# SauersML/genomic_pca

Hardware: AMD Instinct MI355X
Metric: SNPs x samples / sec through rSVD at k=20; max|dPC| vs ref (higher is better)
Workload: dtype i8 (exact: int8 dosages x 4 signed 7-bit fixed-point digit planes of the skinny operand, i32 accumulate, f64 recombination; accuracy >= f32)

## Files before the change

genomic_pca_amd/csrc/gpca_internal.h:

```cpp
#pragma once
#include "../../include/gpca.h"
#include "kernels.h"

#include <dlfcn.h>
#include <hip/hip_runtime.h>

#include <algorithm>
#include <atomic>
#include <chrono>
#include <condition_variable>
#include <deque>
#include <thread>
#include <cmath>
#include <cstdio>
#include <cstdlib>
#include <cstring>
#include <map>
#include <mutex>
#include <string>
#include <vector>

using namespace gpca;

typedef struct ncclComm* ncclComm_t;
// ... 79 lines not shown
    int device = 0;
    int precision = GPCA_PREC_I8_EXACT;
    int storage = GPCA_STORE_INT8;
    int storage_cfg = GPCA_STORE_AUTO;
    int nd_cfg = 0;
    int auto_pin = 0;
    hipStream_t st = nullptr;
    std::string err;

    int64_t M = 0, N = 0, ldg = 0, Mpad = 0;
    int64_t ld8 = 0;
    int64_t cap_rows_pad = 0;
    int64_t cap_stats_pad = 0;
    int8_t* dG = nullptr;
    uint8_t* dG2 = nullptr;
    int64_t ld2 = 0;
    uint32_t pack_flags = 0;

    bool have_stats = false;
    float *d_mu = nullptr, *d_sigma = nullptr, *d_r = nullptr, *d_b = nullptr;
    uint8_t *d_keep = nullptr, *d_reason = nullptr;
    uint32_t *d_counts = nullptr, *d_flags = nullptr;
    int64_t n_pca = 0;
    std::vector<int64_t> pca_rows;
    int64_t* d_pca_rows = nullptr;
    uint32_t flags = 0;

    int k = 0, l = 0, L = 0;
    bool have_rsvd = false;
    float *dQ = nullptr, *dT = nullptr, *dTb = nullptr, *dYpart = nullptr, *d_cpart = nullptr, *d_s32 = nullptr;
    double* h_pin = nullptr;
    int spin_sync = 1;
    int* d_cholflag = nullptr;
    double *d_scratch64 = nullptr, *dY = nullptr, *d_c = nullptr, *d_part64 = nullptr, *dW = nullptr, *dZ = nullptr, *d_s64 = nullptr;
    double* d_tr64 = nullptr; size_t cap_tr64 = 0;
    double* d_scores64 = nullptr; float* d_scores32 = nullptr; float* d_load32 = nullptr; int* d_sign = nullptr;
    double* d_eigres = nullptr;
    double* d_cand_val = nullptr; int64_t* d_cand_idx = nullptr;
    size_t cap_Q = 0, cap_T = 0, cap_Tb = 0, cap_Ypart = 0, cap_cpart = 0, cap_Y = 0, cap_part64 = 0, cap_scores = 0, cap_load = 0;
    std::vector<double> eig, sv;
    GttPlan plan{};
    GqPlan gqplan{};
    Gtt8Plan plan8{};
    int8_t *dQd = nullptr, *dTd = nullptr;
    bool c_fold_pending = false;
    double* d_apart = nullptr; size_t cap_apart = 0; bool apart_valid = false; int64_t apart_parts = 0;
    const double* apart_src[4] = {nullptr, nullptr, nullptr, nullptr};
    float* d_rmax = nullptr; bool rmax_valid = false;
    double* d_amax_run = nullptr;
    double* d_yint = nullptr; size_t cap_yint = 0;
    uint8_t* d_smask = nullptr;
    int64_t n_smask = 0;
    float* d_cw = nullptr; int32_t* d_cfeat0 = nullptr; int c_cmax = 0; int64_t c_R = 0; int c_B = 0;
    int64_t *d_cblk_row0 = nullptr, *d_cblk_row1 = nullptr; int32_t *d_cblk_feat0 = nullptr, *d_cblk_c = nullptr;
    double* dP = nullptr; size_t cap_P = 0;
    float* d_lqr = nullptr; size_t cap_lqr = 0;
    float *d_ones = nullptr, *d_zeros = nullptr; size_t cap_ones = 0, cap_zeros = 0;
    bool loadings_valid = true;
    double* d_status = nullptr;
    double* h_status = nullptr;
    hipEvent_t ev_status = nullptr;
    std::string status_own;
    struct PullLane {
        hipStream_t st = nullptr;
        hipEvent_t dep = nullptr;
        int64_t *d_rows = nullptr, *d_cols = nullptr; float* d_out = nullptr; unsigned long long* d_err = nullptr;
// ... 215 lines not shown
```

genomic_pca_amd/csrc/gpca_residency.cpp:

```cpp
#include "gpca_internal.h"

using namespace gpca;

void free_stats(gpca_handle* h) {
    dfree(h->d_mu); dfree(h->d_sigma); dfree(h->d_r); dfree(h->d_b); dfree(h->d_keep); dfree(h->d_reason);
    dfree(h->d_counts); dfree(h->d_flags); dfree(h->d_pca_rows);
    h->have_stats = false; h->n_pca = 0; h->pca_rows.clear(); h->cap_stats_pad = 0;
}
void free_eigensnp(gpca_handle* h) {
    dfree(h->d_smask); h->n_smask = 0; dfree(h->d_cw); dfree(h->d_cfeat0); dfree(h->d_cblk_row0); dfree(h->d_cblk_row1); dfree(h->d_cblk_feat0); dfree(h->d_cblk_c);
    dfree(h->dP); dfree(h->d_lqr); dfree(h->d_ones); dfree(h->d_zeros);
    h->cap_P = h->cap_lqr = h->cap_ones = h->cap_zeros = 0; h->c_cmax = 0; h->c_R = 0; h->c_B = 0; h->loadings_valid = true;
}
void free_ws(gpca_handle* h) {
    free_eigensnp(h);
    dfree(h->dQ); dfree(h->dT); dfree(h->dTb); dfree(h->dYpart); dfree(h->d_cpart); dfree(h->d_s32); dfree(h->dY); dfree(h->d_c);
    dfree(h->d_part64); dfree(h->dW); dfree(h->dZ); dfree(h->d_s64); dfree(h->d_scores64); dfree(h->d_scores32);
    dfree(h->d_load32); dfree(h->d_sign); dfree(h->d_eigres); dfree(h->d_cand_val); dfree(h->d_cand_idx); dfree(h->d_scratch64); dfree(h->d_tr64); h->cap_tr64 = 0;
    dfree(h->dQd); dfree(h->dTd); dfree(h->dYpart64); dfree(h->d_apart); h->cap_apart = 0; dfree(h->d_cholflag); if (h->h_pin) { (void)hipHostFree(h->h_pin); h->h_pin = nullptr; } dfree(h->d_qscale); dfree(h->d_qinv); dfree(h->d_tscale); dfree(h->d_tinv);
    dfree(h->d_amax_run); dfree(h->d_rmax); h->rmax_valid = false; dfree(h->d_yint); h->cap_yint = 0;
    h->cap_Qd = h->cap_Td = h->cap_Ypart64 = 0;
    h->cap_Q = h->cap_T = h->cap_Tb = h->cap_Ypart = h->cap_cpart = h->cap_Y = h->cap_part64 = h->cap_scores = h->cap_load = 0;
    h->have_rsvd = false;
}
static inline bool host_kind(int kind) { return kind == GPCA_PANEL_HOST_I8 || kind == GPCA_PANEL_HOST_BED || kind == GPCA_PANEL_MAPPED_I8 || kind == GPCA_PANEL_MAPPED_BED; }
static inline bool bed_kind(int kind) { return kind == GPCA_PANEL_HOST_BED || kind == GPCA_PANEL_MAPPED_BED; }
static inline bool mapped_kind(int kind) { return kind == GPCA_PANEL_MAPPED_I8 || kind == GPCA_PANEL_MAPPED_BED; }
static inline double ms_since(std::chrono::steady_clock::time_point t0) {
    return std::chrono::duration<double, std::milli>(std::chrono::steady_clock::now() - t0).count();
}

static void copy_mapped_rows(const Filler& f, int64_t row0, int64_t rows, void* dst) {
    const int64_t w = f.stage_ld;
    const int T = (int)std::max<int64_t>(1, std::min<int64_t>(f.copy_threads, rows * w / (4 << 20)));
    auto part = [&](int t) {
        const int64_t a = rows * t / T, b = rows * (t + 1) / T;
        const uint8_t* src = f.map_base + (size_t)(row0 + a) * (size_t)f.map_ld;
        uint8_t* d = (uint8_t*)dst + (size_t)a * (size_t)w;
        if (f.map_ld == w) memcpy(d, src, (size_t)(b - a) * (size_t)w);
        else for (int64_t r = a; r < b; ++r, src += f.map_ld, d += w) memcpy(d, src, (size_t)w);
    };
    if (T == 1) { part(0); return; }
    std::vector<std::thread> th;
    for (int t = 1; t < T; ++t) th.emplace_back(part, t);
    part(0);
    for (auto& x : th) x.join();
}

static void filler_worker(Filler* f) {
    (void)hipSetDevice(f->device);
    std::unique_lock<std::mutex> lk(f->m);
    for (;;) {
        f->cv.wait(lk, [&] { return f->quit || (!f->jobs.empty() && f->st_state[(size_t)(f->produced % (uint64_t)f->n_stage)] != Filler::kReady); });
        if (f->quit) return;
        const size_t b = (size_t)(f->produced % (uint64_t)f->n_stage);
        const std::pair<int64_t, int64_t> job = f->jobs.front();
// ... 589 lines not shown
```

genomic_pca_amd/csrc/gpca_rsvd.cpp:

```cpp
#include "gpca_internal.h"

using namespace gpca;

static void tred2(int n, double* V, double* d, double* e) {
    for (int j = 0; j < n; ++j) d[j] = V[(n - 1) * n + j];
    for (int i = n - 1; i > 0; --i) {
        double scale = 0.0, h = 0.0;
        for (int k = 0; k < i; ++k) scale += std::fabs(d[k]);
        if (scale == 0.0) {
            e[i] = d[i - 1];
            for (int j = 0; j < i; ++j) { d[j] = V[(i - 1) * n + j]; V[i * n + j] = 0.0; V[j * n + i] = 0.0; }
        } else {
            for (int k = 0; k < i; ++k) { d[k] /= scale; h += d[k] * d[k]; }
            double f = d[i - 1];
            double g = std::sqrt(h);
            if (f > 0) g = -g;
            e[i] = scale * g; h -= f * g; d[i - 1] = f - g;
            for (int j = 0; j < i; ++j) e[j] = 0.0;
            for (int j = 0; j < i; ++j) {
                f = d[j]; V[j * n + i] = f; g = e[j] + V[j * n + j] * f;
                for (int k = j + 1; k <= i - 1; ++k) { g += V[k * n + j] * d[k]; e[k] += V[k * n + j] * f; }
                e[j] = g;
            }
            f = 0.0;
// ... 346 lines not shown
        HIPCHK(hipGetLastError());
    }
    const bool i8 = h->precision == GPCA_PREC_I8_EXACT;
    const int64_t tparts = tail_num_parts(h->ldg);
    const double* csum_part = h->d_part64;
    const double* amax_part = h->d_part64 + tparts * L;
    if (i8 && tparts <= kFinishQFoldMax) {
        for (int hf = 0; hf < L / 32; ++hf) {
            launch_quantize_f64_finishq(h->st, h->dY + 32 * hf, h->N, h->ldg, h->dQd + (size_t)hf * h->ldg * 32 * kDigits, h->storage == GPCA_STORE_2BIT ? 1 : 0, h->nd, L,
                                        csum_part + 32 * hf, amax_part + 32 * hf, tparts, L, h->d_s64 + 32 * hf, h->d_s32 + 32 * hf, h->d_qscale + 32 * hf, h->d_qinv + 32 * hf);
            HIPCHK(hipGetLastError());
        }
        return GPCA_OK;
    }
    launch_finish_q(h->st, csum_part, amax_part, tparts, L, h->d_s64, h->d_s32, i8 ? h->d_qscale : nullptr, i8 ? h->d_qinv : nullptr, h->nd);
    HIPCHK(hipGetLastError());
    if (i8) {
        for (int hf = 0; hf < L / 32; ++hf) {
            launch_quantize_f64_prescaled(h->st, h->dY + 32 * hf, h->N, h->ldg, h->d_qinv + 32 * hf, h->dQd + (size_t)hf * h->ldg * 32 * kDigits,
                                          h->storage == GPCA_STORE_2BIT ? 1 : 0, h->nd, L);
            HIPCHK(hipGetLastError());
        }
    }
    return GPCA_OK;
}

static int ensure_workspace(gpca_handle* h) {
    const int L = h->L;
    const int64_t Npad = h->ldg, M = h->M, N = h->N;
    const int64_t gemm_rows = h->sm.on ? h->sm.panel_rows : h->Mpad;
    h->plan = gtt_plan(h->Mpad, Npad, L, h->gtt_waves_target);
    h->gqplan = k1_plan(h, gemm_rows);
    CHK(ensure(h, h->dQ, h->cap_Q, (size_t)Npad * L));
    CHK(ensure(h, h->dT, h->cap_T, (size_t)h->Mpad * L));
    if (h->precision == GPCA_PREC_F32_MFMA) CHK(ensure(h, h->dTb, h->cap_Tb, (size_t)h->Mpad * L));
    if (h->Mpad > M) HIPCHK(hipMemsetAsync(h->dT + (size_t)M * L, 0, (size_t)(h->Mpad - M) * L * 4, h->st));
    if (h->precision == GPCA_PREC_F32_MFMA) CHK(ensure(h, h->dYpart, h->cap_Ypart, (size_t)h->plan.W * (size_t)Npad * L));
    const int64_t cparts = cpart_capacity(h->gqplan.waves, h->Mpad, L);
    CHK(ensure(h, h->d_cpart, h->cap_cpart, (size_t)cparts));
    CHK(ensure(h, h->dY, h->cap_Y, (size_t)N * L + 16));
    const int64_t p64 = part64_capacity(M, h->Mpad, N, Npad, L);
    CHK(ensure(h, h->d_part64, h->cap_part64, (size_t)p64));
    if (!h->d_c) {
        constexpr size_t LL = (size_t)kMaxSketch * kMaxSketch;
        HIPCHK(hipMalloc((void**)&h->d_c, kMaxSketch * 8)); HIPCHK(hipMalloc((void**)&h->d_s64, kMaxSketch * 8));
        HIPCHK(hipMalloc((void**)&h->d_s32, kMaxSketch * 4)); HIPCHK(hipMalloc((void**)&h->dW, (LL + 16) * 8));
        HIPCHK(hipMalloc((void**)&h->dZ, 2 * LL * 8));
        HIPCHK(hipHostMalloc((void**)&h->h_pin, (3 * LL + 16) * 8, hipHostMallocDefault)); HIPCHK(hipMalloc((void**)&h->d_sign, kMaxSketch * 4));
        HIPCHK(hipMalloc((void**)&h->d_scratch64, (size_t)sum_scratch_capacity(kMaxSketch) * 8));
        HIPCHK(hipMalloc((void**)&h->d_eigres, kEigResCount * 8));
        HIPCHK(hipMalloc((void**)&h->d_cand_val, (size_t)scores_cand_capacity() * 8)); HIPCHK(hipMalloc((void**)&h->d_cand_idx, (size_t)scores_cand_capacity() * 8));
        HIPCHK(hipMalloc((void**)&h->d_cholflag, 4));
    }
    if (h->precision == GPCA_PREC_I8_EXACT) {
        h->plan8 = k2_plan(h, gemm_rows);
        CHK(ensure(h, h->dQd, h->cap_Qd, (size_t)Npad * 32 * kDigits * (size_t)(L / 32)));
        CHK(ensure(h, h->dTd, h->cap_Td, (size_t)h->Mpad * 32 * kDigits * (size_t)(L / 32)));
        int64_t yslices = h->plan8.W;
        if (h->sm.on && h->M % h->sm.panel_rows) yslices = std::max<int64_t>(yslices, k2_plan(h, round_up(h->M % h->sm.panel_rows, kGQRowsPerWave)).W);
        CHK(ensure(h, h->dYpart64, h->cap_Ypart64, (size_t)yslices * (size_t)Npad * 32));
        CHK(ensure(h, h->d_apart, h->cap_apart, (size_t)h->gqplan.waves * 32 * (size_t)(L / 32)));
        if (h->sm.on) CHK(ensure(h, h->d_yint, h->cap_yint, (size_t)N * 32 * (size_t)(L / 32)));
        if (!h->d_qscale) {
            HIPCHK(hipMalloc((void**)&h->d_qscale, kMaxSketch * 8)); HIPCHK(hipMalloc((void**)&h->d_qinv, kMaxSketch * 8));
            HIPCHK(hipMalloc((void**)&h->d_tscale, kMaxSketch * 8)); HIPCHK(hipMalloc((void**)&h->d_tinv, kMaxSketch * 8));
            HIPCHK(hipMalloc((void**)&h->d_amax_run, kMaxSketch * 8));
            HIPCHK(hipMalloc((void**)&h->d_rmax, 4));
        }
    }
    size_t cap2 = h->cap_scores;
    CHK(ensure(h, h->d_scores64, h->cap_scores, (size_t)N * h->k));
    CHK(ensure(h, h->d_scores32, cap2, (size_t)N * h->k));
    CHK(ensure(h, h->d_load32, h->cap_load, (size_t)std::max<int64_t>(h->n_pca, 1) * h->k));
    return GPCA_OK;
}

static int rsvd_preflight(gpca_handle* h, int32_t k, int32_t oversample, int32_t power_iters) {
    if (!have_genotypes(h)) return fail(h, GPCA_ERR_STATE, "gpca_rsvd: no genotypes resident and no panel stream open");
    if (!h->have_stats) return fail(h, GPCA_ERR_STATE, "gpca_rsvd: run gpca_snp_stats or gpca_set_standardization first");
    if (k <= 0) return fail(h, GPCA_ERR_BAD_ARG, "Number of components (-k) must be > 0.");
    if (oversample < 0 || power_iters < 0) return fail(h, GPCA_ERR_BAD_ARG, "gpca_rsvd: negative oversample/power_iters");
    if (h->N < 2) return fail(h, GPCA_ERR_BAD_ARG, "PCA requires at least 2 samples.");
    if (!multi_rank(h) && h->n_pca == 0) return fail(h, GPCA_ERR_BAD_ARG, "PCA requires at least 1 variant (feature), found 0.");
    const int l = k + oversample;
    if (l > kMaxSketch) return fail(h, GPCA_ERR_BAD_ARG, "gpca_rsvd: k + oversample must be <= 128");
    if (l > 64 && h->precision != GPCA_PREC_I8_EXACT)
        return fail(h, GPCA_ERR_BAD_ARG, "gpca_rsvd: sketches wider than 64 columns (k + oversample > 64) run on GPCA_PREC_I8_EXACT; GPCA_PREC_F32_MFMA holds up to 64");
    if (l > h->N || (!multi_rank(h) && l > h->n_pca)) return fail(h, GPCA_ERR_BAD_ARG, "gpca_rsvd: k + oversample exceeds min(samples, PCA SNPs)");
    if (h->flags & 1u) return fail(h, GPCA_ERR_MISSING_GENOTYPE,
        "Unexpected missing genotype (-127i8) in a PCA SNP. This should have been filtered by QC.");
    if (h->flags & 2u) return fail(h, GPCA_ERR_INVALID_GENOTYPE, "a PCA SNP holds a dosage outside {0,1,2}");
    if (h->sm.on && h->precision != GPCA_PREC_I8_EXACT) return fail(h, GPCA_ERR_STATE, "gpca_rsvd: streamed panels need GPCA_PREC_I8_EXACT");
    if (h->precision == GPCA_PREC_I8_EXACT && h->N > ((int64_t)1 << 22))
        return fail(h, GPCA_ERR_BAD_ARG, "gpca_rsvd: the exact-integer path holds up to 4 194 304 samples per matrix (i32 accumulators); use GPCA_PREC_F32_MFMA beyond");
    HIPCHK(hipSetDevice(h->device));
    h->k = k; h->l = l; h->L = l <= 32 ? 32 : (l <= 64 ? 64 : kMaxSketch);
    h->have_rsvd = false;
    CHK(ensure_workspace(h));
    HIPCHK(hipMemsetAsync(h->d_cholflag, 0, 4, h->st));
    return GPCA_OK;
}

static int enqueue_small_eigh(gpca_handle* h, const double* src, int nslices, int zmode, double denom) {
    launch_small_eigh(h->st, src, nslices, h->l, h->L, h->k, zmode, denom, h->d_cholflag, h->dZ, h->d_eigres, nullptr);
    HIPCHK(hipGetLastError());
    return GPCA_OK;
}
static int enqueue_scores_loadings(gpca_handle* h, const float* Xload, bool loadings) {
    const int L = h->L, k = h->k;
    const size_t zk = (size_t)L * k;
    if (L <= 64) {
        launch_scores(h->st, h->dY, h->N, L, h->dZ, k, h->d_scores64, h->d_cand_val, h->d_cand_idx);
        HIPCHK(hipGetLastError());
        launch_scores_sign(h->st, h->d_scores64, h->d_scores32, h->N, k, h->d_cand_val, h->d_cand_idx, scores_num_parts(h->N), h->d_sign);
        HIPCHK(hipGetLastError());
        if (loadings) launch_rightmul_gather_f32(h->st, Xload, h->d_pca_rows, h->n_pca, L, h->dZ + zk, k, h->d_load32, h->d_sign);
    } else {
        launch_rightmul_f64(h->st, h->dY, h->N, L, h->dZ, k, h->d_scores64, (float*)nullptr);
        HIPCHK(hipGetLastError());
        launch_col_sign(h->st, h->d_scores64, h->N, k, h->d_sign);
        launch_scale_cols(h->st, h->d_scores64, h->d_scores32, h->N, k, h->d_sign);
        HIPCHK(hipGetLastError());
        if (loadings) {
            launch_scale_cols(h->st, h->dZ + zk, (float*)nullptr, L, k, h->d_sign);
            launch_rightmul_gather_f32(h->st, Xload, h->d_pca_rows, h->n_pca, L, h->dZ + zk, k, h->d_load32);
        }
    }
    HIPCHK(hipGetLastError());
    return GPCA_OK;
}
static int finish_small_eigh(gpca_handle* h, bool take) {
    double* res = h->h_pin;
    HIPCHK(hipMemcpyAsync(res, h->d_eigres, sizeof(double) * kEigResCount, hipMemcpyDeviceToHost, h->st));
    HIPCHK(stream_wait(h));
    if (!take) return GPCA_OK;
    static_assert(kEigNotConverged == GPCA_ERR_NOT_CONVERGED, "eig_result.h restates the status code");
    const EigVerdict verdict = eig_result_verdict(res, h->l);
    if (verdict.status != 0) return fail(h, verdict.status, verdict.msg);
    h->sv.assign(res + kEigResSv, res + kEigResSv + h->l);
    h->eig.assign(res + kEigResEig, res + kEigResEig + h->k);
    return GPCA_OK;
}

static int call_tail(gpca_handle* h, int zmode, double denom, const float* Xload, int lrc) {
    const bool mr = multi_rank(h);
    const int L = h->L;
    const double* gsrc = h->dW; int gslices = 0;
    auto gram = [&]() -> int {
        const int64_t rows = zmode == 0 ? h->M : h->N;
        const int64_t parts = gram_num_parts(rows);
        if (zmode == 0) launch_gram_f32(h->st, h->dT, rows, L, h->d_part64);
        else launch_gram_f64(h->st, h->dY, rows, L, h->d_part64);
        HIPCHK(hipGetLastError());
        if (mr) launch_sum_partials_f64(h->st, h->d_part64, parts, (int64_t)L * L, h->dW, h->d_scratch64);
        else launch_sum_partials_f64_stage1(h->st, h->d_part64, parts, (int64_t)L * L, h->d_scratch64, &gsrc, &gslices);
        HIPCHK(hipGetLastError());
        return GPCA_OK;
    };
    LOCAL(gram());
    if (mr) {
        h->status_own = h->err;
        status_histogram(h->h_status, lrc);
        if (hipMemcpyAsync(h->dW + (size_t)L * L, h->h_status, 16 * sizeof(double), hipMemcpyHostToDevice, h->st) != hipSuccess && lrc == GPCA_OK)
            lrc = fail(h, GPCA_ERR_HIP, "gpca_rsvd: status copy failed");
        const int xrc = allreduce_f64(h, h->dW, (int64_t)L * L + 16);
        if (xrc != GPCA_OK) return xrc;
    }
// ... 492 lines not shown
```

genomic_pca_amd/csrc/kernels.h:

```cpp
#pragma once
#include <hip/hip_runtime.h>
#include <stdint.h>
#include "eig_result.h"
#include "plan_math.h"

namespace gpca {

struct QcParams { double min_call_rate, min_maf, max_hwe_p; };

struct KernelOpts {
    int gq_phase = -1;
    int gq_chain = 1;
    int gtt_xcd = 1;
};
int init_device_kernels_i8();
int init_device_kernels_common();
int init_device_kernels_eig();

void launch_small_eigh(hipStream_t st, const double* src, int nslices, int n, int L, int k, int zmode, double denom, const int* cholflag,
                       double* Z, double* res, double* Vout);

template <class T>
__host__ __device__ inline constexpr T acc_row(T row0, int e, int h) { return row0 + (e & 3) + 8 * (e >> 2) + 4 * h; }

__host__ __device__ inline int64_t blocked_t_index(int64_t row, int col, int LT) {
    const int64_t group = row >> 4;
    const int w = (int)(row & 15), lt = col >> 5, cc = col & 31;
    return ((group * LT + lt) * 64 + ((w & 1) * 32 + cc)) * 8 + (w >> 1);
}
__host__ __device__ inline int64_t blocked_q_index(int64_t n, int col, int LT) {
    const int64_t chunk = n >> 5;
    const int w = (int)(n & 31), lt = col >> 5, cc = col & 31;
    return ((chunk * LT + lt) * 64 + ((w >> 4) * 32 + cc)) * 16 + (w & 15);
}

void launch_synth(hipStream_t st, int8_t* G, int64_t M, int64_t N, int64_t ld, int64_t snp_offset,
                  uint64_t seed, const uint32_t* d_thresh, int P);
void launch_synth16(hipStream_t st, void* G, int packed, int64_t rows, int64_t N, int64_t ld, int64_t snp0, uint64_t seed,
                    const uint32_t* d_thresh16, int P);
void launch_bed_decode(hipStream_t st, const uint8_t* bed, int64_t bytes_per_row, int8_t* G, int64_t M,
                       int64_t N, int64_t ld);
void launch_snp_stats(hipStream_t st, const int8_t* G, int64_t M, int64_t N, int64_t ld, QcParams qc,
                      float* mu, float* sigma, float* r, float* b, uint8_t* keep, uint8_t* reason,
                      uint32_t* counts, uint32_t* flags);
void launch_set_scale(hipStream_t st, int64_t M, const float* mu, const float* sigma, const uint8_t* keep,
                      float* r, float* b);
void launch_standardize_block(hipStream_t st, const int8_t* G, int64_t ld, const float* mu,
                              const float* sigma, const int64_t* rows, int64_t ns, const int64_t* cols,
                              int64_t nj, float* out, unsigned long long* err_idx);

void launch_omega(hipStream_t st, int64_t M, int64_t Mpad, int l, int L, int64_t snp_offset, uint64_t seed,
                  const float* r, const float* b, float* Tb, float* cpart, double* apart, int blocked = 1, const int64_t* row_ids = nullptr);
// ... 194 lines not shown
```

genomic_pca_amd/csrc/kernels.hip:

```cpp
#include "kernels.h"
#include "philox.hpp"
#include "omega_math.h"

#ifndef GPCA_OMEGA_ABLATE
#define GPCA_OMEGA_ABLATE 0
#endif
namespace gpca {

__device__ const OmegaLnEntry kOmegaLnTable[kOmegaLnEntries] = {
#include "omega_table.inc"
};

typedef float f32x16 __attribute__((ext_vector_type(16)));

#define DEVINL __device__ __forceinline__

__global__ __launch_bounds__(256) void k_synth(int8_t* __restrict__ G, int64_t M, int64_t N, int64_t ld,
                                                int64_t snp_offset, uint64_t seed,
                                                const uint32_t* __restrict__ thresh, int P) {
    const int64_t per_row = ld >> 3;
    const int64_t t = (int64_t)blockIdx.x * 256 + threadIdx.x;
    if (t >= M * per_row) return;
    const int64_t i = t / per_row;
    const int64_t n0 = (t - i * per_row) << 3;
// ... 804 lines not shown
    const int total = (int)rows_here * K;
    float* dst = out32 + n0 * K;
    for (int e = threadIdx.x; e < total; e += 256) dst[e] = osm[(e / K) * KP + (e % K)];
}
static size_t rightmul_lds(int L, int K, bool f32out) { return sizeof(double) * L * K + (f32out ? sizeof(float) * 256 * (size_t)(K | 1) : 0); }
void launch_rightmul_f64(hipStream_t st, const double* X, int64_t rows, int L, const double* Z, int K, double* out64,
                         float* out32) {
    const dim3 grid((unsigned)((rows + 255) / 256)), blk(256);
    const size_t lds = rightmul_lds(L, K, out32 != nullptr);
    if (L == 32) hipLaunchKernelGGL((k_rightmul<double, 32>), grid, blk, lds, st, X, (const int64_t*)nullptr, rows, Z, K, out64, out32);
    else if (L == 64) {
        hipLaunchKernelGGL((k_rightmul<double, 64>), grid, blk, lds, st, X, (const int64_t*)nullptr, rows, Z, K, out64, out32);
    } else launch_rightmul_any_f64(st, X, rows, L, Z, K, out64, out32);
}
template <int L, int NJ>
__global__ __launch_bounds__(256) void k_rightmul_mfma(const float* __restrict__ X, const int64_t* __restrict__ row_ids,
                                                       int64_t nrows, const double* __restrict__ Z, int K,
                                                       float* __restrict__ out32, int64_t tiles_per_wave, const int* __restrict__ sign) {
    constexpr int E = L / 4;
    const int lane = threadIdx.x & 63, wv = threadIdx.x >> 6;
    const int i = lane & 15, kq = lane >> 4;
    double zb[E][NJ];
#pragma unroll
    for (int jt = 0; jt < NJ; ++jt) {
        const int col = 16 * jt + i;
        const double sg = (sign && col < K) ? (double)sign[col] : 1.0;
#pragma unroll
        for (int s2 = 0; s2 < E; ++s2) zb[s2][jt] = col < K ? Z[(E * kq + s2) * K + col] * sg : 0.0;
    }
    __shared__ float osm[4][16 * 64];
    const int64_t ntiles = (nrows + 15) >> 4;
    const int64_t t0 = ((int64_t)blockIdx.x * 4 + wv) * tiles_per_wave;
    const int64_t t1 = (t0 + tiles_per_wave < ntiles) ? t0 + tiles_per_wave : ntiles;
    float xa[E], xn[E];
    auto load_tile = [&](int64_t tile, float (&dst)[E]) {
        const int64_t row = tile * 16 + i;
        const bool valid = row < nrows && tile < t1;
        const int64_t src = valid ? (row_ids ? row_ids[row] : row) : 0;
        const float4* xp = reinterpret_cast<const float4*>(X + src * L + E * kq);
#pragma unroll
        for (int v = 0; v < E / 4; ++v) {
            const float4 q = xp[v];
            dst[4 * v] = valid ? q.x : 0.f; dst[4 * v + 1] = valid ? q.y : 0.f; dst[4 * v + 2] = valid ? q.z : 0.f; dst[4 * v + 3] = valid ? q.w : 0.f;
        }
    };
    if (t0 < t1) load_tile(t0, xa);
    for (int64_t tile = t0; tile < t1; ++tile) {
        load_tile(tile + 1, xn);
        f64x4 acc[NJ];
#pragma unroll
        for (int jt = 0; jt < NJ; ++jt) acc[jt] = f64x4{0.0, 0.0, 0.0, 0.0};
#pragma unroll
        for (int s2 = 0; s2 < E; ++s2) {
            const double a = (double)xa[s2];
#pragma unroll
            for (int jt = 0; jt < NJ; ++jt) acc[jt] = __builtin_amdgcn_mfma_f64_16x16x4f64(a, zb[s2][jt], acc[jt], 0, 0, 0);
        }
#pragma unroll
        for (int jt = 0; jt < NJ; ++jt) {
            const int col = 16 * jt + i;
            if (col < K) {
#pragma unroll
                for (int r = 0; r < 4; ++r) osm[wv][(4 * r + kq) * K + col] = (float)acc[jt][r];
            }
        }
        const int64_t rows_here = (nrows - tile * 16 < 16) ? nrows - tile * 16 : 16;
        float* dst = out32 + tile * 16 * K;
        for (int e = lane; e < (int)rows_here * K; e += 64) dst[e] = osm[wv][e];
#pragma unroll
        for (int s2 = 0; s2 < E; ++s2) xa[s2] = xn[s2];
    }
}
void launch_rightmul_gather_f32(hipStream_t st, const float* X, const int64_t* row_ids, int64_t nrows, int L,
                                const double* Z, int K, float* out32, const int* sign) {
    if (nrows == 0) return;
    if (L > 64) { launch_rightmul_any_gather_f32(st, X, row_ids, nrows, L, Z, K, out32); return; }
    const int64_t ntiles = (nrows + 15) / 16;
    int64_t tpw = ntiles / (4 * 2048);
    if (tpw < 1) tpw = 1;
    const int64_t waves = (ntiles + tpw - 1) / tpw;
    const dim3 grid((unsigned)((waves + 3) / 4)), blk(256);
    const int nj = (K + 15) / 16;
#define GPCA_RM(LL, NN) hipLaunchKernelGGL((k_rightmul_mfma<LL, NN>), grid, blk, 0, st, X, row_ids, nrows, Z, K, out32, tpw, sign)
    if (L == 32) { if (nj == 1) GPCA_RM(32, 1); else if (nj == 2) GPCA_RM(32, 2); else if (nj == 3) GPCA_RM(32, 3); else GPCA_RM(32, 4); }
    else { if (nj == 1) GPCA_RM(64, 1); else if (nj == 2) GPCA_RM(64, 2); else if (nj == 3) GPCA_RM(64, 3); else GPCA_RM(64, 4); }
#undef GPCA_RM
}

template <int L>
__global__ __launch_bounds__(256) void k_scores(const double* __restrict__ X, int64_t nrows, const double* __restrict__ Z, int K,
                                                double* __restrict__ out64, double* __restrict__ cand_val, int64_t* __restrict__ cand_idx) {
    extern __shared__ double zsc[];
    double* tile = zsc + L * K;
    double* win_val = tile + 256 * 17;
    long long* win_idx = reinterpret_cast<long long*>(win_val + 64);
    __shared__ double seg_val[256];
    __shared__ int seg_row[256];
    for (int e = threadIdx.x; e < L * K; e += 256) zsc[e] = Z[e];
    if (threadIdx.x < 64) { win_val[threadIdx.x] = 0.0; win_idx[threadIdx.x] = -1; }
    __syncthreads();
    const int64_t nchunks = (nrows + 255) / 256;
    for (int64_t chunk = blockIdx.x; chunk < nchunks; chunk += gridDim.x) {
        const int64_t n0 = chunk * 256, n = n0 + threadIdx.x;
        const bool live = n < nrows;
        double x[L];
#pragma unroll
        for (int j = 0; j < L; ++j) x[j] = live ? X[n * L + j] : 0.0;
        for (int k0 = 0; k0 < K; k0 += 16) {
            const int kn = K - k0 < 16 ? K - k0 : 16;
            for (int kc = 0; kc < kn; ++kc) {
                double a = 0.0;
#pragma unroll
// ... 270 lines not shown
```

genomic_pca_amd/csrc/small_eig.hip:

```cpp
#include "kernels.h"

#ifndef GPCA_EIG_ABL
#define GPCA_EIG_ABL 0
#endif
#ifndef GPCA_EIG_STAMP
#define GPCA_EIG_STAMP 0
#endif
#if GPCA_EIG_STAMP
__device__ unsigned long long g_eig_stamp[20];
#define EIG_STAMP(SLOT) { if (threadIdx.x == 0) { g_eig_stamp[2 * (SLOT)] = __builtin_amdgcn_s_memrealtime(); g_eig_stamp[2 * (SLOT) + 1] = __builtin_amdgcn_s_memtime(); } }
#define EIG_COUNT(X) (++(X))
#else
#define EIG_STAMP(SLOT)
#define EIG_COUNT(X) ((void)(X))
#endif

namespace gpca {

#define EIGDEV __device__ __forceinline__
EIGDEV double eig_rsqrt(double x) {
    const double y = __builtin_amdgcn_rsq(x);
    const double h = fma(-(x * y), y, 1.0);
    return fma(y * h, fma(0.375, h, 0.5), y);
}
// ... 2 lines not shown
    double r = __builtin_amdgcn_rcp(x);
    r = fma(r, fma(-x, r, 1.0), r);
    return fma(r, fma(-x, r, 1.0), r);
}

constexpr double kJacSkip = 1e-17, kJacDone = 2e-15;
template <int L> struct JacCfg {
    static constexpr int H = L / 2;
    static constexpr int NT = L == 32 ? 256 : 1024;
    static constexpr int NBK = H * H / NT;
    static constexpr int LP = L + 2;
    static constexpr bool DB = L <= 64;
    static constexpr int NBUF = DB ? 4 : 1;
};
EIGDEV int jac_dest(int s, int Le) { return s >= Le ? s : (s == 0 ? 0 : (s == 1 ? (Le > 2 ? 2 : 1) : ((s & 1) ? s - 2 : (s == Le - 2 ? Le - 1 : s + 2)))); }
template <int L> EIGDEV int jac_at(int r, int c) { return r * JacCfg<L>::LP + ((r >> 1) & 1) + c; }

EIGDEV void jac_rot(double app, double a01, double a10, double aqq, double& c, double& s) {
    const double b2 = a01 + a10, dd = aqq - app;
#if GPCA_EIG_ABL & 1
    c = 0.8; s = 0.6; return;
#endif
    const bool live = fabs(b2) > 2.0 * kJacSkip;
    const double sq = live ? fma(dd, dd, b2 * b2) : 1.0;
    const double rinv = eig_rsqrt(sq);
    const double c2 = fabs(dd) * rinv, s2 = (dd >= 0.0 ? b2 : -b2) * rinv;
    const double h = fma(0.5, c2, 0.5);
    const double ci = eig_rsqrt(h);
    c = live ? h * ci : 1.0; s = live ? 0.5 * s2 * ci : 0.0;
}

template <int NT, class GetV>
EIGDEV void eig_emit(GetV getV, double* wsl, int* order, const int* genuine, int slots, int n, int Lw, int k, int zmode, double denom, double unsc,
                     const int* __restrict__ cholflag, int capped, double* __restrict__ Z, double* __restrict__ res, double* __restrict__ Vout, int tid) {
    double wmine = 0.0; int rank = -1;
    if (tid < slots && genuine[tid]) {
        wmine = wsl[tid]; rank = 0;
        for (int t = 0; t < slots; ++t) { const double wt = wsl[t]; if (t != tid && genuine[t] && (wt > wmine || (wt == wmine && t < tid))) ++rank; }
    }
    __syncthreads();
    if (rank >= 0 && rank < n) { order[rank] = tid; wsl[rank] = wmine; }
    __syncthreads();
    for (int j = tid; j < kMaxSketchCols; j += NT) {
        const double w = j < n ? wsl[j] * unsc : 0.0;
        res[kEigResW + j] = w;
        res[kEigResSv + j] = w > 0.0 ? sqrt(w) : 0.0;
        res[kEigResEig + j] = j < k ? w / denom : 0.0;
    }
    if (tid == 0) { res[kEigResFlag] = cholflag ? (double)cholflag[0] : 0.0; res[kEigResFlag + 1] = (double)capped; }
    for (int e0 = tid; e0 < Lw * k; e0 += NT) {
        const int r = e0 / k, c = e0 - r * k;
        double z0 = 0.0, z1 = 0.0;
        if (r < n && c < n) {
            const double x = getV(r, order[c]);
            if (zmode == 0) {
                const double w = wsl[c] * unsc;
                const double sv = w > 0.0 ? sqrt(w) : 0.0;
                z0 = x * sv; z1 = sv > 0.0 ? x / sv : 0.0;
            } else { z0 = x; z1 = x; }
        }
        Z[e0] = z0; Z[(size_t)Lw * k + e0] = z1;
    }
    EIG_STAMP(4)
    if (Vout)
        for (int e0 = tid; e0 < n * n; e0 += NT) { const int r = e0 / n, c = e0 - r * n; Vout[e0] = getV(r, order[c]); }
}

template <int L>
__global__ __launch_bounds__(JacCfg<L>::NT) void k_small_eigh(const double* __restrict__ src, int nslices, int n, int Lw, int k, int zmode, double denom,
                                                             const int* __restrict__ cholflag, double* __restrict__ Z, double* __restrict__ res,
                                                             double* __restrict__ Vout) {
    using C = JacCfg<L>;
    constexpr int H = C::H, NT = C::NT, NBK = C::NBK, LP = C::LP, BUF = L * LP;
    extern __shared__ double eig_sm[];
    __shared__ double wsl[128];
    __shared__ int order[128], genuine[128];
    __shared__ double redmax[NT];
    const int tid = threadIdx.x;
#if GPCA_EIG_STAMP
    if (tid == 0) { g_eig_stamp[10] = 0; g_eig_stamp[11] = 0; }
#endif
    EIG_STAMP(0)
    const int S = nslices > 0 ? nslices : 1;
    const size_t LL = (size_t)Lw * Lw;
    double* buf0 = eig_sm;
    for (int e0 = tid; e0 < BUF; e0 += NT) buf0[e0] = 0.0;
    __syncthreads();
    for (int e0 = tid; e0 < n * n; e0 += 4 * NT) {
        const double* p[4];
        double acc[4] = {0.0, 0.0, 0.0, 0.0};
#pragma unroll
        for (int q = 0; q < 4; ++q) { const int e1 = e0 + NT * q; const int e2 = e1 < n * n ? e1 : e0; p[q] = src + (size_t)(e2 / n) * Lw + (e2 % n); }
        for (int s0 = 0; s0 < S; s0 += 8) {
            double v[4][8];
#pragma unroll
            for (int u = 0; u < 8; ++u) {
                const int sl = s0 + u < S ? s0 + u : s0;
#pragma unroll
                for (int q = 0; q < 4; ++q) v[q][u] = p[q][sl * LL];
            }
#pragma unroll
            for (int u = 0; u < 8; ++u)
#pragma unroll
// ... 139 lines not shown
    static constexpr int RING = 512;
    static constexpr int NCONS = L / 64;
    static constexpr int kDoubles = L * L + 6 * L + 64 + 2 * RING;
    static constexpr size_t kBytes = sizeof(double) * kDoubles + sizeof(int) * (RING + 16);
};
template <int L> EIGDEV int ql_at(int r, int c) { return r * L + ((c + r) & (L - 1)); }
EIGDEV int ql_tag(int seq) { return (((seq >> 9) + 1) & 0xffff) << 12; }
template <int CTRL, int ROWMASK> EIGDEV double eig_dpp0(double v) {
    const int hi = __builtin_amdgcn_update_dpp(0, __double2hiint(v), CTRL, ROWMASK, 0xf, true);
    const int lo = __builtin_amdgcn_update_dpp(0, __double2loint(v), CTRL, ROWMASK, 0xf, true);
    return __hiloint2double(hi, lo);
}
EIGDEV double eig_lane(double v, int i) {
    return __hiloint2double(__builtin_amdgcn_readlane(__double2hiint(v), i), __builtin_amdgcn_readlane(__double2loint(v), i));
}
EIGDEV double wave_sum(double x) {
    x += eig_dpp0<0x111, 0xf>(x); x += eig_dpp0<0x112, 0xf>(x); x += eig_dpp0<0x114, 0xf>(x); x += eig_dpp0<0x118, 0xf>(x);
    x += eig_dpp0<0x142, 0xa>(x); x += eig_dpp0<0x143, 0xc>(x);
    return eig_lane(x, 63);
}
EIGDEV double oct_sum(double x) {
    x += eig_dpp0<0xb1, 0xf>(x);
    x += eig_dpp0<0x4e, 0xf>(x);
    x += eig_dpp0<0x141, 0xf>(x);
    return x;
}
EIGDEV double wave_max(double x) { for (int o = 32; o > 0; o >>= 1) x = fmax(x, __shfl_xor(x, o)); return x; }
constexpr int kQlFirst = 1 << 30, kQlLast = 1 << 29, kQlDoneFlag = 1 << 28, kQlIndex = 0xff, kQlTagMask = 0xffff << 12;
constexpr int kQlSpinCap = 4000000;
enum { kQlTail0 = 2, kQlTail1 = 3, kQlGaveUp = 4 };

template <int L>
__global__ __launch_bounds__(QlCfg<L>::NT) void k_small_eigh_ql(const double* __restrict__ src, int nslices, int n, int Lw, int k, int zmode, double denom,
                                                                const int* __restrict__ cholflag, double* __restrict__ Z, double* __restrict__ res,
                                                                double* __restrict__ Vout) {
    using C = QlCfg<L>;
    constexpr int NT = C::NT, RING = C::RING;
    extern __shared__ double eig_sm[];
    typedef __attribute__((address_space(3))) double lds_d;
    typedef __attribute__((address_space(3))) int lds_i;
    typedef double v2d __attribute__((ext_vector_type(2)));
    typedef __attribute__((address_space(3))) v2d lds_d2;
    lds_d* A = (lds_d*)eig_sm;
    lds_d* de = A + L * L;
    lds_d* vv = A + L * L + 2 * L;
    lds_d* pp = vv + L;
    lds_d* ww = pp + L;
    lds_d* bb = ww + L;
    lds_d* red = bb + L;
    volatile lds_d2* ringcs = (volatile lds_d2*)(red + 64);
    volatile lds_i* ringi = (volatile lds_i*)(red + 64 + 2 * RING);
    volatile lds_i* ctrl = ringi + RING;
    __shared__ double wsl[128];
    __shared__ int order[128], genuine[128];
    const int tid = threadIdx.x, lane = tid & 63, wave = tid >> 6;
    EIG_STAMP(0)
    const int S = nslices > 0 ? nslices : 1;
    const size_t LL = (size_t)Lw * Lw;
    for (int e0 = tid; e0 < L * L; e0 += NT) A[e0] = 0.0;
    if (tid < 16) ctrl[tid] = 0;
    for (int e0 = tid; e0 < RING; e0 += NT) ringi[e0] = 0;
    if (tid < 128) { order[tid] = 0; genuine[tid] = tid < n; }
    __syncthreads();
    for (int e0 = tid; e0 < n * n; e0 += NT) {
        const int r = e0 / n, c = e0 - r * n;
        const double* p0 = src + (size_t)r * Lw + c;
        double acc = 0.0;
// ... 271 lines not shown
                carry = hi;
            }
            tail += len; EIG_COUNT(batches);
            if ((tail & 63) < len && lane == 0) ctrl[kQlTail0 + wave - 1] = tail;
        }
#if GPCA_EIG_STAMP
        if (wave == 1 && lane == 0) { g_eig_stamp[13] = (unsigned long long)batches; g_eig_stamp[14] = (unsigned long long)empty_polls; }
#endif
        (void)batches; (void)empty_polls;
    }
    __syncthreads();
    capped = ctrl[kQlGaveUp] != 0 || (wave == 0 && capped);
    if (wave == 0 && lane == 0 && capped) ctrl[kQlGaveUp] = 1;
    __syncthreads();
    capped = ctrl[kQlGaveUp];
    EIG_STAMP(3)
    if (tid < 128) wsl[tid] = tid < n ? de[2 * tid] : 0.0;
    __syncthreads();
    eig_emit<NT>([&](int r, int slot) { return A[ql_at<L>(r, slot)]; }, wsl, order, genuine, L, n, Lw, k, zmode, denom, unsc, cholflag, capped, Z, res, Vout, tid);
}

template <int L> static size_t small_eigh_lds() { return sizeof(double) * (size_t)L * JacCfg<L>::LP * JacCfg<L>::NBUF; }
#ifndef GPCA_EIG_QL
#define GPCA_EIG_QL 1
#endif
int init_device_kernels_eig() {
    hipError_t e = hipFuncSetAttribute(reinterpret_cast<const void*>(k_small_eigh<128>), hipFuncAttributeMaxDynamicSharedMemorySize, (int)small_eigh_lds<128>());
    if (e == hipSuccess) e = hipFuncSetAttribute(reinterpret_cast<const void*>(k_small_eigh_ql<128>), hipFuncAttributeMaxDynamicSharedMemorySize, (int)QlCfg<128>::kBytes);
    if (e == hipSuccess) e = hipFuncSetAttribute(reinterpret_cast<const void*>(k_small_eigh_ql<64>), hipFuncAttributeMaxDynamicSharedMemorySize, (int)QlCfg<64>::kBytes);
    if (e == hipSuccess) e = hipFuncSetAttribute(reinterpret_cast<const void*>(k_small_eigh<64>), hipFuncAttributeMaxDynamicSharedMemorySize, (int)small_eigh_lds<64>());
    if (e == hipSuccess) e = hipFuncSetAttribute(reinterpret_cast<const void*>(k_small_eigh<32>), hipFuncAttributeMaxDynamicSharedMemorySize, (int)small_eigh_lds<32>());
    return (int)e;
}
void launch_small_eigh(hipStream_t st, const double* src, int nslices, int n, int L, int k, int zmode, double denom, const int* cholflag,
                       double* Z, double* res, double* Vout) {
    if (n <= 32) hipLaunchKernelGGL(k_small_eigh<32>, dim3(1), dim3(JacCfg<32>::NT), small_eigh_lds<32>(), st, src, nslices, n, L, k, zmode, denom, cholflag, Z, res, Vout);
    else if (GPCA_EIG_QL == 2 && n <= 64) hipLaunchKernelGGL(k_small_eigh_ql<64>, dim3(1), dim3(QlCfg<64>::NT), QlCfg<64>::kBytes, st, src, nslices, n, L, k, zmode, denom, cholflag, Z, res, Vout);
    else if (GPCA_EIG_QL && n > 64) hipLaunchKernelGGL(k_small_eigh_ql<128>, dim3(1), dim3(QlCfg<128>::NT), QlCfg<128>::kBytes, st, src, nslices, n, L, k, zmode, denom, cholflag, Z, res, Vout);
    else if (n <= 64) hipLaunchKernelGGL(k_small_eigh<64>, dim3(1), dim3(JacCfg<64>::NT), small_eigh_lds<64>(), st, src, nslices, n, L, k, zmode, denom, cholflag, Z, res, Vout);
    else hipLaunchKernelGGL(k_small_eigh<128>, dim3(1), dim3(JacCfg<128>::NT), small_eigh_lds<128>(), st, src, nslices, n, L, k, zmode, denom, cholflag, Z, res, Vout);
}

}
```

Before: 965.6 billion.

## Skip redundant per-call memsets and deepen gather-rightmul prefetch

The eig kernel now clears the Cholesky flag itself after reading it, so the per-call memset of that flag can be skipped once a completed eig run is known. The zero-fill of T's padding rows is cached and redone only when the buffer or its shape changes. The gather right-multiply kernel now prefetches two tiles ahead instead of one and uses a different tiles-per-wave split. These cut small launches per call and hide load latency, at the cost of extra state tracking and registers.

```diff
diff --git a/genomic_pca_amd/csrc/gpca_internal.h b/genomic_pca_amd/csrc/gpca_internal.h
--- a/genomic_pca_amd/csrc/gpca_internal.h
+++ b/genomic_pca_amd/csrc/gpca_internal.h
@@ -135,6 +135,8 @@
     double* h_pin = nullptr;
     int spin_sync = 1;
     int* d_cholflag = nullptr;
+    bool cholflag_zero = false, cholflag_eig_enqueued = false;
+    int64_t tpad_M = -1, tpad_Mpad = -1; int tpad_L = 0;
     double *d_scratch64 = nullptr, *dY = nullptr, *d_c = nullptr, *d_part64 = nullptr, *dW = nullptr, *dZ = nullptr, *d_s64 = nullptr;
     double* d_tr64 = nullptr; size_t cap_tr64 = 0;
     double* d_scores64 = nullptr; float* d_scores32 = nullptr; float* d_load32 = nullptr; int* d_sign = nullptr;
diff --git a/genomic_pca_amd/csrc/gpca_residency.cpp b/genomic_pca_amd/csrc/gpca_residency.cpp
--- a/genomic_pca_amd/csrc/gpca_residency.cpp
+++ b/genomic_pca_amd/csrc/gpca_residency.cpp
@@ -22,6 +22,7 @@
     h->cap_Qd = h->cap_Td = h->cap_Ypart64 = 0;
     h->cap_Q = h->cap_T = h->cap_Tb = h->cap_Ypart = h->cap_cpart = h->cap_Y = h->cap_part64 = h->cap_scores = h->cap_load = 0;
     h->have_rsvd = false;
+    h->cholflag_zero = false; h->tpad_M = -1;
 }
 static inline bool host_kind(int kind) { return kind == GPCA_PANEL_HOST_I8 || kind == GPCA_PANEL_HOST_BED || kind == GPCA_PANEL_MAPPED_I8 || kind == GPCA_PANEL_MAPPED_BED; }
 static inline bool bed_kind(int kind) { return kind == GPCA_PANEL_HOST_BED || kind == GPCA_PANEL_MAPPED_BED; }
diff --git a/genomic_pca_amd/csrc/gpca_rsvd.cpp b/genomic_pca_amd/csrc/gpca_rsvd.cpp
--- a/genomic_pca_amd/csrc/gpca_rsvd.cpp
+++ b/genomic_pca_amd/csrc/gpca_rsvd.cpp
@@ -402,9 +402,17 @@
     h->plan = gtt_plan(h->Mpad, Npad, L, h->gtt_waves_target);
     h->gqplan = k1_plan(h, gemm_rows);
     CHK(ensure(h, h->dQ, h->cap_Q, (size_t)Npad * L));
-    CHK(ensure(h, h->dT, h->cap_T, (size_t)h->Mpad * L));
+    {
+        const float* T_was = h->dT; const size_t cap_was = h->cap_T;
+        CHK(ensure(h, h->dT, h->cap_T, (size_t)h->Mpad * L));
+        if (h->dT != T_was || h->cap_T != cap_was) h->tpad_M = -1;
+    }
     if (h->precision == GPCA_PREC_F32_MFMA) CHK(ensure(h, h->dTb, h->cap_Tb, (size_t)h->Mpad * L));
-    if (h->Mpad > M) HIPCHK(hipMemsetAsync(h->dT + (size_t)M * L, 0, (size_t)(h->Mpad - M) * L * 4, h->st));
+    if (h->Mpad > M && !(h->tpad_M == M && h->tpad_Mpad == h->Mpad && h->tpad_L == L)) {
+        h->tpad_M = -1;
+        HIPCHK(hipMemsetAsync(h->dT + (size_t)M * L, 0, (size_t)(h->Mpad - M) * L * 4, h->st));
+        h->tpad_M = M; h->tpad_Mpad = h->Mpad; h->tpad_L = L;
+    }
     if (h->precision == GPCA_PREC_F32_MFMA) CHK(ensure(h, h->dYpart, h->cap_Ypart, (size_t)h->plan.W * (size_t)Npad * L));
     const int64_t cparts = cpart_capacity(h->gqplan.waves, h->Mpad, L);
     CHK(ensure(h, h->d_cpart, h->cap_cpart, (size_t)cparts));
@@ -467,13 +475,15 @@
     h->k = k; h->l = l; h->L = l <= 32 ? 32 : (l <= 64 ? 64 : kMaxSketch);
     h->have_rsvd = false;
     CHK(ensure_workspace(h));
-    HIPCHK(hipMemsetAsync(h->d_cholflag, 0, 4, h->st));
+    if (!h->cholflag_zero) HIPCHK(hipMemsetAsync(h->d_cholflag, 0, 4, h->st));
+    h->cholflag_zero = false; h->cholflag_eig_enqueued = false;
     return GPCA_OK;
 }
 
 static int enqueue_small_eigh(gpca_handle* h, const double* src, int nslices, int zmode, double denom) {
     launch_small_eigh(h->st, src, nslices, h->l, h->L, h->k, zmode, denom, h->d_cholflag, h->dZ, h->d_eigres, nullptr);
     HIPCHK(hipGetLastError());
+    h->cholflag_eig_enqueued = true;
     return GPCA_OK;
 }
 static int enqueue_scores_loadings(gpca_handle* h, const float* Xload, bool loadings) {
@@ -503,6 +513,7 @@
     double* res = h->h_pin;
     HIPCHK(hipMemcpyAsync(res, h->d_eigres, sizeof(double) * kEigResCount, hipMemcpyDeviceToHost, h->st));
     HIPCHK(stream_wait(h));
+    if (h->cholflag_eig_enqueued) h->cholflag_zero = true;
     if (!take) return GPCA_OK;
     static_assert(kEigNotConverged == GPCA_ERR_NOT_CONVERGED, "eig_result.h restates the status code");
     const EigVerdict verdict = eig_result_verdict(res, h->l);
diff --git a/genomic_pca_amd/csrc/kernels.h b/genomic_pca_amd/csrc/kernels.h
--- a/genomic_pca_amd/csrc/kernels.h
+++ b/genomic_pca_amd/csrc/kernels.h
@@ -17,7 +17,7 @@
 int init_device_kernels_common();
 int init_device_kernels_eig();
 
-void launch_small_eigh(hipStream_t st, const double* src, int nslices, int n, int L, int k, int zmode, double denom, const int* cholflag,
+void launch_small_eigh(hipStream_t st, const double* src, int nslices, int n, int L, int k, int zmode, double denom, int* cholflag,
                        double* Z, double* res, double* Vout);
 
 template <class T>
diff --git a/genomic_pca_amd/csrc/kernels.hip b/genomic_pca_amd/csrc/kernels.hip
--- a/genomic_pca_amd/csrc/kernels.hip
+++ b/genomic_pca_amd/csrc/kernels.hip
@@ -860,21 +860,31 @@
     const int64_t ntiles = (nrows + 15) >> 4;
     const int64_t t0 = ((int64_t)blockIdx.x * 4 + wv) * tiles_per_wave;
     const int64_t t1 = (t0 + tiles_per_wave < ntiles) ? t0 + tiles_per_wave : ntiles;
-    float xa[E], xn[E];
-    auto load_tile = [&](int64_t tile, float (&dst)[E]) {
+    float xa[E], xb[E], xc[E];
+    auto tile_src = [&](int64_t tile) -> int64_t {
         const int64_t row = tile * 16 + i;
-        const bool valid = row < nrows && tile < t1;
-        const int64_t src = valid ? (row_ids ? row_ids[row] : row) : 0;
-        const float4* xp = reinterpret_cast<const float4*>(X + src * L + E * kq);
+        if (!(row < nrows && tile < t1)) return -1;
+        return row_ids ? row_ids[row] : row;
+    };
+    auto load_tile = [&](int64_t src, float (&dst)[E]) {
+        const bool valid = src >= 0;
+        const float4* xp = reinterpret_cast<const float4*>(X + (valid ? src : 0) * L + E * kq);
 #pragma unroll
         for (int v = 0; v < E / 4; ++v) {
             const float4 q = xp[v];
             dst[4 * v] = valid ? q.x : 0.f; dst[4 * v + 1] = valid ? q.y : 0.f; dst[4 * v + 2] = valid ? q.z : 0.f; dst[4 * v + 3] = valid ? q.w : 0.f;
         }
     };
-    if (t0 < t1) load_tile(t0, xa);
+    int64_t src2 = -1;
+    if (t0 < t1) {
+        load_tile(tile_src(t0), xa);
+        load_tile(tile_src(t0 + 1), xb);
+        src2 = tile_src(t0 + 2);
+    }
     for (int64_t tile = t0; tile < t1; ++tile) {
-        load_tile(tile + 1, xn);
+        const int64_t src3 = tile_src(tile + 3);
+        load_tile(src2, xc);
+        src2 = src3;
         f64x4 acc[NJ];
 #pragma unroll
         for (int jt = 0; jt < NJ; ++jt) acc[jt] = f64x4{0.0, 0.0, 0.0, 0.0};
@@ -896,7 +906,7 @@
         float* dst = out32 + tile * 16 * K;
         for (int e = lane; e < (int)rows_here * K; e += 64) dst[e] = osm[wv][e];
 #pragma unroll
-        for (int s2 = 0; s2 < E; ++s2) xa[s2] = xn[s2];
+        for (int s2 = 0; s2 < E; ++s2) { xa[s2] = xb[s2]; xb[s2] = xc[s2]; }
     }
 }
 void launch_rightmul_gather_f32(hipStream_t st, const float* X, const int64_t* row_ids, int64_t nrows, int L,
@@ -904,8 +914,7 @@
     if (nrows == 0) return;
     if (L > 64) { launch_rightmul_any_gather_f32(st, X, row_ids, nrows, L, Z, K, out32); return; }
     const int64_t ntiles = (nrows + 15) / 16;
-    int64_t tpw = ntiles / (4 * 2048);
-    if (tpw < 1) tpw = 1;
+    const int64_t tpw = std::max<int64_t>(1, (ntiles + 4 * 1024 - 1) / (4 * 1024));
     const int64_t waves = (ntiles + tpw - 1) / tpw;
     const dim3 grid((unsigned)((waves + 3) / 4)), blk(256);
     const int nj = (K + 15) / 16;
diff --git a/genomic_pca_amd/csrc/small_eig.hip b/genomic_pca_amd/csrc/small_eig.hip
--- a/genomic_pca_amd/csrc/small_eig.hip
+++ b/genomic_pca_amd/csrc/small_eig.hip
@@ -58,7 +58,7 @@
 
 template <int NT, class GetV>
 EIGDEV void eig_emit(GetV getV, double* wsl, int* order, const int* genuine, int slots, int n, int Lw, int k, int zmode, double denom, double unsc,
-                     const int* __restrict__ cholflag, int capped, double* __restrict__ Z, double* __restrict__ res, double* __restrict__ Vout, int tid) {
+                     int* __restrict__ cholflag, int capped, double* __restrict__ Z, double* __restrict__ res, double* __restrict__ Vout, int tid) {
     double wmine = 0.0; int rank = -1;
     if (tid < slots && genuine[tid]) {
         wmine = wsl[tid]; rank = 0;
@@ -73,7 +73,10 @@
         res[kEigResSv + j] = w > 0.0 ? sqrt(w) : 0.0;
         res[kEigResEig + j] = j < k ? w / denom : 0.0;
     }
-    if (tid == 0) { res[kEigResFlag] = cholflag ? (double)cholflag[0] : 0.0; res[kEigResFlag + 1] = (double)capped; }
+    if (tid == 0) {
+        res[kEigResFlag] = cholflag ? (double)cholflag[0] : 0.0; res[kEigResFlag + 1] = (double)capped;
+        if (cholflag) cholflag[0] = 0;
+    }
     for (int e0 = tid; e0 < Lw * k; e0 += NT) {
         const int r = e0 / k, c = e0 - r * k;
         double z0 = 0.0, z1 = 0.0;
@@ -94,7 +97,7 @@
 
 template <int L>
 __global__ __launch_bounds__(JacCfg<L>::NT) void k_small_eigh(const double* __restrict__ src, int nslices, int n, int Lw, int k, int zmode, double denom,
-                                                             const int* __restrict__ cholflag, double* __restrict__ Z, double* __restrict__ res,
+                                                             int* __restrict__ cholflag, double* __restrict__ Z, double* __restrict__ res,
                                                              double* __restrict__ Vout) {
     using C = JacCfg<L>;
     constexpr int H = C::H, NT = C::NT, NBK = C::NBK, LP = C::LP, BUF = L * LP;
@@ -300,7 +303,7 @@
 
 template <int L>
 __global__ __launch_bounds__(QlCfg<L>::NT) void k_small_eigh_ql(const double* __restrict__ src, int nslices, int n, int Lw, int k, int zmode, double denom,
-                                                                const int* __restrict__ cholflag, double* __restrict__ Z, double* __restrict__ res,
+                                                                int* __restrict__ cholflag, double* __restrict__ Z, double* __restrict__ res,
                                                                 double* __restrict__ Vout) {
     using C = QlCfg<L>;
     constexpr int NT = C::NT, RING = C::RING;
@@ -638,7 +641,7 @@
     if (e == hipSuccess) e = hipFuncSetAttribute(reinterpret_cast<const void*>(k_small_eigh<32>), hipFuncAttributeMaxDynamicSharedMemorySize, (int)small_eigh_lds<32>());
     return (int)e;
 }
-void launch_small_eigh(hipStream_t st, const double* src, int nslices, int n, int L, int k, int zmode, double denom, const int* cholflag,
+void launch_small_eigh(hipStream_t st, const double* src, int nslices, int n, int L, int k, int zmode, double denom, int* cholflag,
                        double* Z, double* res, double* Vout) {
     if (n <= 32) hipLaunchKernelGGL(k_small_eigh<32>, dim3(1), dim3(JacCfg<32>::NT), small_eigh_lds<32>(), st, src, nslices, n, L, k, zmode, denom, cholflag, Z, res, Vout);
     else if (GPCA_EIG_QL == 2 && n <= 64) hipLaunchKernelGGL(k_small_eigh_ql<64>, dim3(1), dim3(QlCfg<64>::NT), QlCfg<64>::kBytes, st, src, nslices, n, L, k, zmode, denom, cholflag, Z, res, Vout);
```

Result: no change. 967.3 billion (median of 5 runs) (+0.2%).
